# anuragranj/cc

Measured on AMD Instinct MI355X. Metric: train images/sec (832x256, 5-frame sample, 6-scale CC step), higher is better.
Workload: dtype f32; 1 GPU; full CC: DispResNet6+PoseNetB6+MaskNet6+Back2Future, all losses; per_gpu_batch=4, global_batch=4, height=256, width=832, scales=6, frames=5, parallelism=dp1, hipgraph=True, trained_nets=all, rccl_ranks=1, dead_occlusion_decoders_elided=False, net_streams=2, pipeline=per_network, grad_chunks=False, deterministic=True

## Files before the change

### cc_amd/csrc/wgrad_thin.hip

```cpp
#include <stdio.h>
#include <type_traits>
#include <stdlib.h>
#include "cc_common.h"
#include "conv_internal.h"
#include "cc_tools.h"

namespace {

typedef float f32x4 __attribute__((ext_vector_type(4)));

constexpr int THIN_NW = 4;

struct WT {
    const float* a; const float* x; float* ws;
    int B, M, AH, AW; long a_bs;
    int Cin, IH, IW; long x_bs;
    int R, nxc, units, upb, npb, ngc, ngt, swz;
};

template <int S, int SI, int PAD, int TR>
struct ThinCfg {
    static constexpr int PQ = (PAD + 3) / 4;
    static constexpr int IMAX = SI * 3 + S - 1 - PAD + 4 * PQ;
    static constexpr int NQ = IMAX / 4 + 1;
    static constexpr int TS = TR * S;
};

template <int S, int SI, int PAD, int TR, int DBG>
__device__ __forceinline__ void wgrad_thin_body(const WT& g, const int bx_, const int by_) {
    typedef ThinCfg<S, SI, PAD, TR> C;
    constexpr int PQ = C::PQ, NQ = C::NQ, TS = C::TS;
    __shared__ float red[TS * 256];
    const int lane = threadIdx.x & 63;
    const int wave = __builtin_amdgcn_readfirstlane((int)(threadIdx.x >> 6));
    const int i = lane & 15, k = lane >> 4;
    int combo = by_;
    const int tg = combo % g.ngt;
    combo /= g.ngt;
    const int cg = combo % g.ngc, mg = combo / g.ngc;
    const int r0 = tg * TR;
    const int m = mg * 16 + i, c = cg * 16 + i;
    const bool mok = m < g.M, cok = c < g.Cin;
    const float* __restrict__ abase = g.a + (long)(mok ? m : 0) * g.AH * g.AW;
    const float* __restrict__ xbase = g.x + (long)(cok ? c : 0) * g.IH * g.IW;

    f32x4 acc[TR][S];
#pragma unroll
    for (int tr = 0; tr < TR; tr++)
#pragma unroll
        for (int s = 0; s < S; s++) acc[tr][s] = (f32x4){0.f, 0.f, 0.f, 0.f};

    const int pb = (g.swz ? ((bx_ & 7) * (g.npb >> 3) + (bx_ >> 3)) : bx_);
    const int u0 = pb * g.upb;
    const int u1 = (u0 + g.upb < g.units) ? (u0 + g.upb) : g.units;

    constexpr int KEEP = (TR > SI) ? TR - SI : 0;
    float4 An;
    float4 Wn[TR][NQ], Wc[TR][NQ];
    auto issue = [&](auto T0, int b, int y, int xc, float4& A, float4 (&W)[TR][NQ]) {
        constexpr int t0 = decltype(T0)::value;
        const int x0 = xc * 16 + 4 * k;
        const int xa = (x0 < g.AW) ? x0 : 0;
        A = *(const float4*)(abase + (unsigned)(b * (int)g.a_bs + y * g.AW + xa));
        const unsigned xb = (unsigned)(b * (int)g.x_bs);
#pragma unroll
        for (int tr = t0; tr < TR; tr++) {
            int iy = y * SI + r0 + tr - PAD;
            iy = iy < 0 ? 0 : (iy >= g.IH ? g.IH - 1 : iy);
            const unsigned xr = xb + (unsigned)(iy * g.IW);
#pragma unroll
            for (int q = 0; q < NQ; q++) {
                int col = SI * x0 - 4 * PQ + 4 * q;
                col = (col < 0 || col >= g.IW) ? 0 : col;
                W[tr][q] = *(const float4*)(xbase + (xr + (unsigned)col));
            }
        }
    };

    const int ngx = (g.nxc + THIN_NW - 1) / THIN_NW;
    int u = u0;
    const int ue = u1;
    if (u < ue) {
        int nb, ny, nxcpos;
        {
            const int colu = u / g.AH;
            ny = u - colu * g.AH;
            nb = colu / ngx;
            nxcpos = (colu - nb * ngx) * THIN_NW + wave;
        }
        typedef std::integral_constant<int, 0> ALL;
        typedef std::integral_constant<int, KEEP> NEW;
        issue(ALL(), nb, ny, nxcpos, An, Wn);
        bool fresh = true;
        for (; u < ue; u++) {
            const float4 Ac = An;
            if (fresh) {
#pragma unroll
                for (int tr = 0; tr < TR; tr++)
#pragma unroll
                    for (int q = 0; q < NQ; q++) Wc[tr][q] = Wn[tr][q];
            } else {
#pragma unroll
                for (int tr = 0; tr < TR; tr++)
#pragma unroll
                    for (int q = 0; q < NQ; q++) Wc[tr][q] = (tr < KEEP) ? Wc[tr + (TR - KEEP)][q] : Wn[tr][q];
            }
            const int y = ny, xc = nxcpos;
            if (u + 1 < ue) {
                fresh = false;
                if (++ny == g.AH) {
                    ny = 0;
                    fresh = true;
                    nxcpos += THIN_NW;
                    if (nxcpos - wave >= g.nxc) { nxcpos = wave; nb++; }
                }
                if (DBG != 2) {
                    if (fresh) issue(ALL(), nb, ny, nxcpos, An, Wn);
                    else issue(NEW(), nb, ny, nxcpos, An, Wn);
                }
            }

            const int x0 = xc * 16 + 4 * k;
            const bool aok = mok && (x0 < g.AW);
            float a4[4];
            a4[0] = aok ? Ac.x : 0.f;
            a4[1] = aok ? Ac.y : 0.f;
            a4[2] = aok ? Ac.z : 0.f;
            a4[3] = aok ? Ac.w : 0.f;
#pragma unroll
            for (int tr = 0; tr < TR; tr++) {
                const int iy = y * SI + r0 + tr - PAD;
                const bool rok = cok && (r0 + tr < g.R) && iy >= 0 && iy < g.IH;
                float w[NQ * 4];
#pragma unroll
                for (int q = 0; q < NQ; q++) {
                    const int col = SI * x0 - 4 * PQ + 4 * q;
                    const bool ok = rok && col >= 0 && col < g.IW;
                    w[4 * q + 0] = ok ? Wc[tr][q].x : 0.f;
                    w[4 * q + 1] = ok ? Wc[tr][q].y : 0.f;
                    w[4 * q + 2] = ok ? Wc[tr][q].z : 0.f;
                    w[4 * q + 3] = ok ? Wc[tr][q].w : 0.f;
                }
                if (DBG == 1) {
#pragma unroll
                    for (int s = 0; s < S; s++)
#pragma unroll
                        for (int j = 0; j < 4; j++) acc[tr][s][j] += a4[j] * w[SI * j + s - PAD + 4 * PQ];
                    continue;
                }
#pragma unroll
                for (int j = 0; j < 4; j++)
#pragma unroll
                    for (int s = 0; s < S; s++)
                        acc[tr][s] = __builtin_amdgcn_mfma_f32_16x16x4f32(a4[j], w[SI * j + s - PAD + 4 * PQ], acc[tr][s], 0, 0, 0);
            }
        }
    }

#pragma unroll 1
    for (int wv = 0; wv < THIN_NW; wv++) {
        if (wave == wv) {
#pragma unroll
            for (int tr = 0; tr < TR; tr++)
#pragma unroll
                for (int s = 0; s < S; s++)
#pragma unroll
                    for (int r = 0; r < 4; r++) {
                        const int idx = ((tr * S + s) * 4 + r) * 64 + lane;
                        const float v = acc[tr][s][r];
                        red[idx] = (wv == 0) ? v : (red[idx] + v);
                    }
        }
        __syncthreads();
    }
    float* __restrict__ slab = g.ws + ((long)by_ * g.npb + pb) * (TS * 256);
    for (int e = threadIdx.x; e < TS * 256; e += 64 * THIN_NW) {
        const int t = e >> 8, mc = e & 255, mm = mc >> 4, cc_ = mc & 15;
        slab[e] = red[(t * 4 + (mm & 3)) * 64 + (mm >> 2) * 16 + cc_];
    }
}


template <int S, int SI, int PAD, int TR, int DBG = 0>
__global__ __launch_bounds__(64 * THIN_NW) void k_wgrad_thin(WT g) {
    wgrad_thin_body<S, SI, PAD, TR, DBG>(g, (int)blockIdx.x, (int)blockIdx.y);
}

constexpr int THIN_MAXP = 24;
struct WTM { WT p[THIN_MAXP]; int blk_end[THIN_MAXP]; int n; };
template <int S, int SI, int PAD, int TR>
__global__ __launch_bounds__(64 * THIN_NW) void k_wgrad_thin_multi(WTM a) {
    int k = 0, first = 0;
#pragma unroll 1
    for (int q = 0; q + 1 < a.n; q++)
        if ((int)blockIdx.x >= a.blk_end[q]) { k = q + 1; first = a.blk_end[q]; }
#if defined(__HIP_DEVICE_COMPILE__) && !defined(CC_HIPEMU)
    const WT& g = *(reinterpret_cast<const WT*>((const char*)__builtin_amdgcn_kernarg_segment_ptr() + offsetof(WTM, p)) + k);
#else
    const WT& g = a.p[k];
#endif
    const int b = (int)blockIdx.x - first;
    const int by = b / g.npb;
    wgrad_thin_body<S, SI, PAD, TR, 0>(g, b - by * g.npb, by);
}


int env_int(const char* name, int dflt) { return cctools::env_int(name, dflt); }

struct ThinPlan {
    bool ok;
    int kind, TR, ngm, ngc, ngt, nxc, units, upb, npb, TS;
    size_t ws_floats;
};

enum { K_3_1 = 0, K_3_2, K_7_2, K_7_1, K_1_1, K_5_2, K_4_2, K_1_2, K_NONE };

ThinPlan plan_thin(int B, int M, int AH, int AW, int Cin, int R, int S, int si) {
    ThinPlan p = {};
    p.kind = K_NONE;
    if (R != S || env_int("CC_NO_WGRAD_THIN", 0)) return p;
    if (S == 3 && si == 1) { p.kind = K_3_1; p.TR = 3; }
    else if (S == 3 && si == 2) { p.kind = K_3_2; p.TR = 3; }
    else if (S == 7 && si == 2) { p.kind = K_7_2; p.TR = 2; }
    else if (S == 7 && si == 1) { p.kind = K_7_1; p.TR = 2; }
    else if (S == 1 && si == 1) { p.kind = K_1_1; p.TR = 1; }
    else if (S == 5 && si == 2) { p.kind = K_5_2; p.TR = 3; }
    else if (S == 4 && si == 2) { p.kind = K_4_2; p.TR = 4; }
    else if (S == 1 && si == 2) { p.kind = K_1_2; p.TR = 1; }
    else return p;
    p.ngm = (M + 15) / 16;
    p.ngc = (Cin + 15) / 16;
    const long P = (long)B * AH * AW;
    if ((AW & 3) || p.ngm * p.ngc > env_int("CC_WGRAD_THIN_MAXCOMBO", 15) || P < env_int("CC_WGRAD_THIN_MINPIX", 8192) ||
        (S == 7 && Cin < 8)) return p;
    p.ngt = (R + p.TR - 1) / p.TR;
    p.TS = p.TR * S;
    p.nxc = (AW + 15) / 16;
    const long units = (long)B * AH * ((p.nxc + THIN_NW - 1) / THIN_NW);
    if (units > (1l << 30)) return p;
    p.units = (int)units;
    long npb = units / env_int("CC_WGRAD_THIN_UPB", 8);
    const long cap = env_int("CC_WGRAD_THIN_NPB", 256);
    npb = npb < 1 ? 1 : (npb > cap ? cap : npb);
    p.upb = (int)((units + npb - 1) / npb);
    p.npb = (p.units + p.upb - 1) / p.upb;
    if (p.npb >= 64) p.npb = ((p.npb + 7) / 8) * 8;
    p.ws_floats = (size_t)p.ngm * p.ngc * p.ngt * p.npb * p.TS * 256;
    p.ok = true;
    return p;
}

template <int S, int SI, int PAD, int TR>
void launch_thin(const WT& g, dim3 grid, hipStream_t s) {
    hipLaunchKernelGGL(HIP_KERNEL_NAME(k_wgrad_thin<S, SI, PAD, TR>), grid, dim3(64 * THIN_NW), 0, s, g);
}

template <int S, int SI, int PAD, int TR>
void launch_thin_multi(const WTM& m, unsigned blocks, hipStream_t s) {
    hipLaunchKernelGGL(HIP_KERNEL_NAME(k_wgrad_thin_multi<S, SI, PAD, TR>), dim3(blocks), dim3(64 * THIN_NW), 0, s, m);
}

constexpr int THIN_PARK_CAP = 96;
struct ThinParkedOne { WT g; int kind, ncombo; double gflop; };
struct ThinParked { bool on; int n; ThinParkedOne d[THIN_PARK_CAP]; };
thread_local ThinParked g_thin_parked = {};

void launch_thin_kind(int kind, const WT& g, dim3 grid, hipStream_t s) {
    switch (kind) {
        case K_3_1: launch_thin<3, 1, 1, 3>(g, grid, s); break;
        case K_3_2: launch_thin<3, 2, 1, 3>(g, grid, s); break;
        case K_7_2: launch_thin<7, 2, 3, 2>(g, grid, s); break;
        case K_7_1: launch_thin<7, 1, 3, 2>(g, grid, s); break;
        case K_1_1: launch_thin<1, 1, 0, 1>(g, grid, s); break;
        case K_5_2: launch_thin<5, 2, 2, 3>(g, grid, s); break;
        case K_1_2: launch_thin<1, 2, 0, 1>(g, grid, s); break;
        default: launch_thin<4, 2, 1, 4>(g, grid, s); break;
    }
}

void launch_thin_multi_kind(int kind, const WTM& m, unsigned blocks, hipStream_t s) {
    switch (kind) {
        case K_3_1: launch_thin_multi<3, 1, 1, 3>(m, blocks, s); break;
        case K_3_2: launch_thin_multi<3, 2, 1, 3>(m, blocks, s); break;
        case K_7_2: launch_thin_multi<7, 2, 3, 2>(m, blocks, s); break;
        case K_7_1: launch_thin_multi<7, 1, 3, 2>(m, blocks, s); break;
        case K_1_1: launch_thin_multi<1, 1, 0, 1>(m, blocks, s); break;
        case K_5_2: launch_thin_multi<5, 2, 2, 3>(m, blocks, s); break;
        case K_1_2: launch_thin_multi<1, 2, 0, 1>(m, blocks, s); break;
        default: launch_thin_multi<4, 2, 1, 4>(m, blocks, s); break;
    }
}

}

namespace ccint {

bool wgrad_thin_park(bool on) {
    const bool was = g_thin_parked.on;
    g_thin_parked.on = on && !env_int("CC_NO_WGRAD_THIN_LIST", 0);
    return was;
}

bool wgrad_thin_parking() { return g_thin_parked.on; }

double wgrad_thin_parked_gflop() {
    double gf = 0;
    for (int i = 0; i < g_thin_parked.n; i++) gf += g_thin_parked.d[i].gflop;
    return gf;
}

void wgrad_thin_flush(hipStream_t s) {
    ThinParked& P = g_thin_parked;
    for (int kind = 0; kind < K_NONE && P.n > 0; kind++) {
        int i = 0;
        while (i < P.n) {
            WTM m = {};
            long blk = 0;
            int last = -1;
            for (; i < P.n && m.n < THIN_MAXP; i++) {
                if (P.d[i].kind != kind) continue;
                const long nb = (long)P.d[i].g.npb * P.d[i].ncombo;
                if (m.n && blk + nb >= (1l << 31)) break;
                m.p[m.n] = P.d[i].g;
                blk += nb;
                m.blk_end[m.n] = (int)blk;
                m.n++;
                last = i;
            }
            if (!m.n) break;
            if (env_int("CC_WGRAD_THIN_TRACE", 0)) fprintf(stderr, "[wgrad_thin_multi] kind %d: %d problems, %ld workgroups\n", kind, m.n, blk);
            if (m.n == 1) launch_thin_kind(kind, P.d[last].g, dim3((unsigned)P.d[last].g.npb, (unsigned)P.d[last].ncombo), s);
            else launch_thin_multi_kind(kind, m, (unsigned)blk, s);
        }
    }
    P.n = 0;
}

size_t wgrad_thin_ws_floats(int B, int M, int AH, int AW, int Cin, int R, int S, int si) {
    const ThinPlan p = plan_thin(B, M, AH, AW, Cin, R, S, si);
    return p.ok ? p.ws_floats : 0;
}

bool wgrad_thin_launch(const float* a, const float* x, float* gw, float* ws, int B, int M, int AH, int AW, long a_bs, int Cin,
                       int IH, int IW, long x_bs, int R, int S, int si, int pad, long o_sm, long o_sc, int accumulate, hipStream_t s,
                       RedSink* sink) {
    const ThinPlan p = plan_thin(B, M, AH, AW, Cin, R, S, si);
    if (!p.ok || (IW & 3) || (a_bs & 3) || (x_bs & 3) || (((uintptr_t)a | (uintptr_t)x) & 15)) return false;
    if ((long)B * a_bs >= (1l << 31) || (long)B * x_bs >= (1l << 31)) return false;
    static const int want_pad[] = {1, 1, 3, 3, 0, 2, 1, 0};
    if (pad != want_pad[p.kind]) return false;
    WT g = {};
    g.a = a; g.x = x; g.ws = ws;
    g.B = B; g.M = M; g.AH = AH; g.AW = AW; g.a_bs = a_bs; g.Cin = Cin; g.IH = IH; g.IW = IW; g.x_bs = x_bs;
    g.R = R; g.nxc = p.nxc; g.units = p.units; g.upb = p.upb; g.npb = p.npb; g.ngc = p.ngc; g.ngt = p.ngt;
    g.swz = (p.npb % 8 == 0 && p.npb >= 64 && !env_int("CC_WGRAD_THIN_NOSWZ", 0)) ? 1 : 0;
    const int ncombo = p.ngm * p.ngc * p.ngt;
    if (env_int("CC_WGRAD_THIN_TRACE", 0))
        fprintf(stderr, "[wgrad_thin] kind %d M %d Cin %d A %dx%d X %dx%d npb %d upb %d combos %d\n", p.kind, M, Cin, AH, AW, IH, IW,
                p.npb, p.upb, ncombo);
    dim3 grid((unsigned)p.npb, (unsigned)ncombo);
    if (g_thin_parked.on && sink && g_thin_parked.n < THIN_PARK_CAP) {
        ThinParkedOne& d = g_thin_parked.d[g_thin_parked.n++];
        d.g = g; d.kind = p.kind; d.ncombo = ncombo;
        d.gflop = 2e-9 * B * AH * AW * (double)M * Cin * R * S;
        const long rdp[RD_LONGS] = {2, (long)ws, (long)gw, p.npb, accumulate, o_sm, o_sc, p.TS, S, p.TR, p.ngc, p.ngt, M, Cin, R, ncombo};
        (void)wgrad_reduce_emit(sink, rdp, 1, s);
        return true;
    }
    switch (p.kind) {
        case K_3_1: {
            const int dbg = env_int("CC_WGRAD_THIN_DBG", 0);
            if (dbg == 1) hipLaunchKernelGGL(HIP_KERNEL_NAME(k_wgrad_thin<3, 1, 1, 3, 1>), grid, dim3(64 * THIN_NW), 0, s, g);
            else if (dbg == 2) hipLaunchKernelGGL(HIP_KERNEL_NAME(k_wgrad_thin<3, 1, 1, 3, 2>), grid, dim3(64 * THIN_NW), 0, s, g);
            else launch_thin<3, 1, 1, 3>(g, grid, s);
            break;
        }
        case K_3_2: launch_thin<3, 2, 1, 3>(g, grid, s); break;
        case K_7_2: launch_thin<7, 2, 3, 2>(g, grid, s); break;
        case K_7_1: launch_thin<7, 1, 3, 2>(g, grid, s); break;
        case K_1_1: launch_thin<1, 1, 0, 1>(g, grid, s); break;
        case K_5_2: launch_thin<5, 2, 2, 3>(g, grid, s); break;
        case K_1_2: launch_thin<1, 2, 0, 1>(g, grid, s); break;
        default: launch_thin<4, 2, 1, 4>(g, grid, s); break;
    }
    const long rd[RD_LONGS] = {2, (long)ws, (long)gw, p.npb, accumulate, o_sm, o_sc, p.TS, S, p.TR, p.ngc, p.ngt, M, Cin, R, ncombo};
    (void)wgrad_reduce_emit(sink, rd, 1, s);
    return true;
}

void wgrad_thin_name(int B, int M, int AH, int AW, int Cin, int IH, int IW, int R, int S, int si, int pad, char* out, int cap) {
    out[0] = 0;
    const ThinPlan p = plan_thin(B, M, AH, AW, Cin, R, S, si);
    static const int want_pad[] = {1, 1, 3, 3, 0, 2, 1, 0};
    static const int tr[] = {3, 3, 2, 2, 1, 3, 4, 1};
    if (!p.ok || (IW & 3) || pad != want_pad[p.kind]) return;
    snprintf(out, cap, "k_wgrad_thin<%d, %d, %d, %d>", S, si, pad, tr[p.kind]);
}

}
```

Before: 248.1 images/s.

## Process two dY channel groups per wave in thin wgrad to reuse input loads

The thin weight-gradient kernel now lets each workgroup handle two 16-channel output groups (GM=2) for selected kernel kinds. The input rows loaded for the MFMA B-operand are shared across both groups, and the grid is halved in the M dimension. It also restructures row prefetch so kept rows are reloaded only at column changes. This trades higher register pressure, more accumulators and a serialized two-pass LDS reduction for fewer redundant global loads of x.

```diff
diff --git a/cc_amd/csrc/wgrad_thin.hip b/cc_amd/csrc/wgrad_thin.hip
--- a/cc_amd/csrc/wgrad_thin.hip
+++ b/cc_amd/csrc/wgrad_thin.hip
@@ -26,55 +26,54 @@
     static constexpr int TS = TR * S;
 };
 
-template <int S, int SI, int PAD, int TR, int DBG>
-__device__ __forceinline__ void wgrad_thin_body(const WT& g, const int bx_, const int by_) {
+template <int S, int SI, int PAD, int TR, int DBG, int GM, int NG>
+__device__ __forceinline__ void wgrad_thin_units(const WT& g, const int mg0, const int cg, const int r0, const int u0, const int u1,
+                                                 f32x4 (&acc)[GM][TR][S]) {
     typedef ThinCfg<S, SI, PAD, TR> C;
-    constexpr int PQ = C::PQ, NQ = C::NQ, TS = C::TS;
-    __shared__ float red[TS * 256];
+    constexpr int PQ = C::PQ, NQ = C::NQ;
     const int lane = threadIdx.x & 63;
     const int wave = __builtin_amdgcn_readfirstlane((int)(threadIdx.x >> 6));
     const int i = lane & 15, k = lane >> 4;
-    int combo = by_;
-    const int tg = combo % g.ngt;
-    combo /= g.ngt;
-    const int cg = combo % g.ngc, mg = combo / g.ngc;
-    const int r0 = tg * TR;
-    const int m = mg * 16 + i, c = cg * 16 + i;
-    const bool mok = m < g.M, cok = c < g.Cin;
-    const float* __restrict__ abase = g.a + (long)(mok ? m : 0) * g.AH * g.AW;
+    const int c = cg * 16 + i;
+    const bool cok = c < g.Cin;
     const float* __restrict__ xbase = g.x + (long)(cok ? c : 0) * g.IH * g.IW;
-
-    f32x4 acc[TR][S];
-#pragma unroll
-    for (int tr = 0; tr < TR; tr++)
-#pragma unroll
-        for (int s = 0; s < S; s++) acc[tr][s] = (f32x4){0.f, 0.f, 0.f, 0.f};
-
-    const int pb = (g.swz ? ((bx_ & 7) * (g.npb >> 3) + (bx_ >> 3)) : bx_);
-    const int u0 = pb * g.upb;
-    const int u1 = (u0 + g.upb < g.units) ? (u0 + g.upb) : g.units;
+    bool mok[NG];
+    const float* __restrict__ abase[NG];
+#pragma unroll
+    for (int gi = 0; gi < NG; gi++) {
+        const int m = (mg0 + gi) * 16 + i;
+        mok[gi] = m < g.M;
+        abase[gi] = g.a + (long)(mok[gi] ? m : 0) * g.AH * g.AW;
+    }
 
     constexpr int KEEP = (TR > SI) ? TR - SI : 0;
-    float4 An;
-    float4 Wn[TR][NQ], Wc[TR][NQ];
-    auto issue = [&](auto T0, int b, int y, int xc, float4& A, float4 (&W)[TR][NQ]) {
-        constexpr int t0 = decltype(T0)::value;
+    constexpr int NR = TR - KEEP;
+    float4 An[NG];
+    float4 Wn[NR][NQ], Wc[TR][NQ];
+    auto issue_row = [&](int tr, int b, int y, int xc, float4 (&W)[NQ]) {
+        const int x0 = xc * 16 + 4 * k;
+        int iy = y * SI + r0 + tr - PAD;
+        iy = iy < 0 ? 0 : (iy >= g.IH ? g.IH - 1 : iy);
+        const unsigned xr = (unsigned)(b * (int)g.x_bs) + (unsigned)(iy * g.IW);
+#pragma unroll
+        for (int q = 0; q < NQ; q++) {
+            int col = SI * x0 - 4 * PQ + 4 * q;
+            col = (col < 0 || col >= g.IW) ? 0 : col;
+            W[q] = *(const float4*)(xbase + (xr + (unsigned)col));
+        }
+    };
+    auto issue = [&](int b, int y, int xc) {
         const int x0 = xc * 16 + 4 * k;
         const int xa = (x0 < g.AW) ? x0 : 0;
-        A = *(const float4*)(abase + (unsigned)(b * (int)g.a_bs + y * g.AW + xa));
-        const unsigned xb = (unsigned)(b * (int)g.x_bs);
-#pragma unroll
-        for (int tr = t0; tr < TR; tr++) {
-            int iy = y * SI + r0 + tr - PAD;
-            iy = iy < 0 ? 0 : (iy >= g.IH ? g.IH - 1 : iy);
-            const unsigned xr = xb + (unsigned)(iy * g.IW);
-#pragma unroll
-            for (int q = 0; q < NQ; q++) {
-                int col = SI * x0 - 4 * PQ + 4 * q;
-                col = (col < 0 || col >= g.IW) ? 0 : col;
-                W[tr][q] = *(const float4*)(xbase + (xr + (unsigned)col));
-            }
-        }
+        const unsigned ao = (unsigned)(b * (int)g.a_bs + y * g.AW + xa);
+#pragma unroll
+        for (int gi = 0; gi < NG; gi++) An[gi] = *(const float4*)(abase[gi] + ao);
+#pragma unroll
+        for (int tr = KEEP; tr < TR; tr++) issue_row(tr, b, y, xc, Wn[tr - KEEP]);
+    };
+    auto issue_keep = [&](int b, int y, int xc) {
+#pragma unroll
+        for (int tr = 0; tr < KEEP; tr++) issue_row(tr, b, y, xc, Wc[tr + NR]);
     };
 
     const int ngx = (g.nxc + THIN_NW - 1) / THIN_NW;
@@ -88,45 +87,38 @@
             nb = colu / ngx;
             nxcpos = (colu - nb * ngx) * THIN_NW + wave;
         }
-        typedef std::integral_constant<int, 0> ALL;
-        typedef std::integral_constant<int, KEEP> NEW;
-        issue(ALL(), nb, ny, nxcpos, An, Wn);
-        bool fresh = true;
+        issue_keep(nb, ny, nxcpos);
+        issue(nb, ny, nxcpos);
         for (; u < ue; u++) {
-            const float4 Ac = An;
-            if (fresh) {
-#pragma unroll
-                for (int tr = 0; tr < TR; tr++)
-#pragma unroll
-                    for (int q = 0; q < NQ; q++) Wc[tr][q] = Wn[tr][q];
-            } else {
-#pragma unroll
-                for (int tr = 0; tr < TR; tr++)
-#pragma unroll
-                    for (int q = 0; q < NQ; q++) Wc[tr][q] = (tr < KEEP) ? Wc[tr + (TR - KEEP)][q] : Wn[tr][q];
-            }
+            float4 Ac[NG];
+#pragma unroll
+            for (int gi = 0; gi < NG; gi++) Ac[gi] = An[gi];
+#pragma unroll
+            for (int tr = 0; tr < TR; tr++)
+#pragma unroll
+                for (int q = 0; q < NQ; q++) Wc[tr][q] = (tr < KEEP) ? Wc[tr + NR][q] : Wn[tr - KEEP][q];
             const int y = ny, xc = nxcpos;
+            bool fresh = false;
             if (u + 1 < ue) {
-                fresh = false;
                 if (++ny == g.AH) {
                     ny = 0;
                     fresh = true;
                     nxcpos += THIN_NW;
                     if (nxcpos - wave >= g.nxc) { nxcpos = wave; nb++; }
                 }
-                if (DBG != 2) {
-                    if (fresh) issue(ALL(), nb, ny, nxcpos, An, Wn);
-                    else issue(NEW(), nb, ny, nxcpos, An, Wn);
-                }
+                if (DBG != 2) issue(nb, ny, nxcpos);
             }
 
             const int x0 = xc * 16 + 4 * k;
-            const bool aok = mok && (x0 < g.AW);
-            float a4[4];
-            a4[0] = aok ? Ac.x : 0.f;
-            a4[1] = aok ? Ac.y : 0.f;
-            a4[2] = aok ? Ac.z : 0.f;
-            a4[3] = aok ? Ac.w : 0.f;
+            float a4[NG][4];
+#pragma unroll
+            for (int gi = 0; gi < NG; gi++) {
+                const bool aok = mok[gi] && (x0 < g.AW);
+                a4[gi][0] = aok ? Ac[gi].x : 0.f;
+                a4[gi][1] = aok ? Ac[gi].y : 0.f;
+                a4[gi][2] = aok ? Ac[gi].z : 0.f;
+                a4[gi][3] = aok ? Ac[gi].w : 0.f;
+            }
 #pragma unroll
             for (int tr = 0; tr < TR; tr++) {
                 const int iy = y * SI + r0 + tr - PAD;
@@ -141,54 +133,94 @@
                     w[4 * q + 2] = ok ? Wc[tr][q].z : 0.f;
                     w[4 * q + 3] = ok ? Wc[tr][q].w : 0.f;
                 }
-                if (DBG == 1) {
+#pragma unroll
+                for (int gi = 0; gi < NG; gi++) {
+                    if (DBG == 1) {
+#pragma unroll
+                        for (int s = 0; s < S; s++)
+#pragma unroll
+                            for (int j = 0; j < 4; j++) acc[gi][tr][s][j] += a4[gi][j] * w[SI * j + s - PAD + 4 * PQ];
+                        continue;
+                    }
+#pragma unroll
+                    for (int j = 0; j < 4; j++)
+#pragma unroll
+                        for (int s = 0; s < S; s++)
+                            acc[gi][tr][s] =
+                                __builtin_amdgcn_mfma_f32_16x16x4f32(a4[gi][j], w[SI * j + s - PAD + 4 * PQ], acc[gi][tr][s], 0, 0, 0);
+                }
+            }
+            if (KEEP > 0 && DBG != 2 && fresh) issue_keep(nb, ny, nxcpos);
+        }
+    }
+}
+
+template <int S, int SI, int PAD, int TR, int DBG, int GM>
+__device__ __forceinline__ void wgrad_thin_body(const WT& g, const int bx_, const int by_) {
+    typedef ThinCfg<S, SI, PAD, TR> C;
+    constexpr int TS = C::TS;
+    static_assert(GM == 1 || GM == 2, "one or two dY channel groups per wave");
+    __shared__ float red[TS * 256];
+    const int lane = threadIdx.x & 63;
+    const int wave = __builtin_amdgcn_readfirstlane((int)(threadIdx.x >> 6));
+    int combo = by_;
+    const int tg = combo % g.ngt;
+    combo /= g.ngt;
+    const int cg = combo % g.ngc, mg0 = (combo / g.ngc) * GM;
+    const int ng = (GM > 1 && mg0 + 1 < (g.M + 15) / 16) ? GM : 1;
+
+    f32x4 acc[GM][TR][S];
+#pragma unroll
+    for (int gi = 0; gi < GM; gi++)
+#pragma unroll
+        for (int tr = 0; tr < TR; tr++)
+#pragma unroll
+            for (int s = 0; s < S; s++) acc[gi][tr][s] = (f32x4){0.f, 0.f, 0.f, 0.f};
+
+    const int pb = (g.swz ? ((bx_ & 7) * (g.npb >> 3) + (bx_ >> 3)) : bx_);
+    const int u0 = pb * g.upb;
+    const int u1 = (u0 + g.upb < g.units) ? (u0 + g.upb) : g.units;
+
+    if (GM > 1 && ng == GM) wgrad_thin_units<S, SI, PAD, TR, DBG, GM, GM>(g, mg0, cg, tg * TR, u0, u1, acc);
+    else wgrad_thin_units<S, SI, PAD, TR, DBG, GM, 1>(g, mg0, cg, tg * TR, u0, u1, acc);
+
+#pragma unroll
+    for (int gi = 0; gi < GM; gi++) {
+        if (gi >= ng) break;
+        if (gi) __syncthreads();
+#pragma unroll 1
+        for (int wv = 0; wv < THIN_NW; wv++) {
+            if (wave == wv) {
+#pragma unroll
+                for (int tr = 0; tr < TR; tr++)
 #pragma unroll
                     for (int s = 0; s < S; s++)
 #pragma unroll
-                        for (int j = 0; j < 4; j++) acc[tr][s][j] += a4[j] * w[SI * j + s - PAD + 4 * PQ];
-                    continue;
-                }
-#pragma unroll
-                for (int j = 0; j < 4; j++)
-#pragma unroll
-                    for (int s = 0; s < S; s++)
-                        acc[tr][s] = __builtin_amdgcn_mfma_f32_16x16x4f32(a4[j], w[SI * j + s - PAD + 4 * PQ], acc[tr][s], 0, 0, 0);
+                        for (int r = 0; r < 4; r++) {
+                            const int idx = ((tr * S + s) * 4 + r) * 64 + lane;
+                            const float v = acc[gi][tr][s][r];
+                            red[idx] = (wv == 0) ? v : (red[idx] + v);
+                        }
             }
-        }
-    }
-
-#pragma unroll 1
-    for (int wv = 0; wv < THIN_NW; wv++) {
-        if (wave == wv) {
-#pragma unroll
-            for (int tr = 0; tr < TR; tr++)
-#pragma unroll
-                for (int s = 0; s < S; s++)
-#pragma unroll
-                    for (int r = 0; r < 4; r++) {
-                        const int idx = ((tr * S + s) * 4 + r) * 64 + lane;
-                        const float v = acc[tr][s][r];
-                        red[idx] = (wv == 0) ? v : (red[idx] + v);
-                    }
-        }
-        __syncthreads();
-    }
-    float* __restrict__ slab = g.ws + ((long)by_ * g.npb + pb) * (TS * 256);
-    for (int e = threadIdx.x; e < TS * 256; e += 64 * THIN_NW) {
-        const int t = e >> 8, mc = e & 255, mm = mc >> 4, cc_ = mc & 15;
-        slab[e] = red[(t * 4 + (mm & 3)) * 64 + (mm >> 2) * 16 + cc_];
-    }
-}
-
-
-template <int S, int SI, int PAD, int TR, int DBG = 0>
+            __syncthreads();
+        }
+        float* __restrict__ slab = g.ws + ((((long)(mg0 + gi) * g.ngc + cg) * g.ngt + tg) * g.npb + pb) * (TS * 256);
+        for (int e = threadIdx.x; e < TS * 256; e += 64 * THIN_NW) {
+            const int t = e >> 8, mc = e & 255, mm = mc >> 4, cc_ = mc & 15;
+            slab[e] = red[(t * 4 + (mm & 3)) * 64 + (mm >> 2) * 16 + cc_];
+        }
+    }
+}
+
+
+template <int S, int SI, int PAD, int TR, int DBG = 0, int GM = 1>
 __global__ __launch_bounds__(64 * THIN_NW) void k_wgrad_thin(WT g) {
-    wgrad_thin_body<S, SI, PAD, TR, DBG>(g, (int)blockIdx.x, (int)blockIdx.y);
+    wgrad_thin_body<S, SI, PAD, TR, DBG, GM>(g, (int)blockIdx.x, (int)blockIdx.y);
 }
 
 constexpr int THIN_MAXP = 24;
 struct WTM { WT p[THIN_MAXP]; int blk_end[THIN_MAXP]; int n; };
-template <int S, int SI, int PAD, int TR>
+template <int S, int SI, int PAD, int TR, int GM = 1>
 __global__ __launch_bounds__(64 * THIN_NW) void k_wgrad_thin_multi(WTM a) {
     int k = 0, first = 0;
 #pragma unroll 1
@@ -201,7 +233,7 @@
 #endif
     const int b = (int)blockIdx.x - first;
     const int by = b / g.npb;
-    wgrad_thin_body<S, SI, PAD, TR, 0>(g, b - by * g.npb, by);
+    wgrad_thin_body<S, SI, PAD, TR, 0, GM>(g, b - by * g.npb, by);
 }
 
 
@@ -250,44 +282,54 @@
     return p;
 }
 
+constexpr int THIN_GM_KINDS = (1 << K_3_1) | (1 << K_3_2) | (1 << K_1_2);
+int thin_gm(int kind) {
+    if (env_int("CC_WGRAD_THIN_GM", 2) < 2) return 1;
+    return ((env_int("CC_WGRAD_THIN_GM_KINDS", THIN_GM_KINDS) >> kind) & 1) ? 2 : 1;
+}
+
+int thin_rows(int ngm, int ngc, int ngt, int gm) { return ((ngm + gm - 1) / gm) * ngc * ngt; }
+
 template <int S, int SI, int PAD, int TR>
-void launch_thin(const WT& g, dim3 grid, hipStream_t s) {
-    hipLaunchKernelGGL(HIP_KERNEL_NAME(k_wgrad_thin<S, SI, PAD, TR>), grid, dim3(64 * THIN_NW), 0, s, g);
+void launch_thin(const WT& g, dim3 grid, int gm, hipStream_t s) {
+    if (gm == 2) hipLaunchKernelGGL(HIP_KERNEL_NAME(k_wgrad_thin<S, SI, PAD, TR, 0, 2>), grid, dim3(64 * THIN_NW), 0, s, g);
+    else hipLaunchKernelGGL(HIP_KERNEL_NAME(k_wgrad_thin<S, SI, PAD, TR, 0, 1>), grid, dim3(64 * THIN_NW), 0, s, g);
 }
 
 template <int S, int SI, int PAD, int TR>
-void launch_thin_multi(const WTM& m, unsigned blocks, hipStream_t s) {
-    hipLaunchKernelGGL(HIP_KERNEL_NAME(k_wgrad_thin_multi<S, SI, PAD, TR>), dim3(blocks), dim3(64 * THIN_NW), 0, s, m);
+void launch_thin_multi(const WTM& m, unsigned blocks, int gm, hipStream_t s) {
+    if (gm == 2) hipLaunchKernelGGL(HIP_KERNEL_NAME(k_wgrad_thin_multi<S, SI, PAD, TR, 2>), dim3(blocks), dim3(64 * THIN_NW), 0, s, m);
+    else hipLaunchKernelGGL(HIP_KERNEL_NAME(k_wgrad_thin_multi<S, SI, PAD, TR, 1>), dim3(blocks), dim3(64 * THIN_NW), 0, s, m);
 }
 
 constexpr int THIN_PARK_CAP = 96;
-struct ThinParkedOne { WT g; int kind, ncombo; double gflop; };
+struct ThinParkedOne { WT g; int kind, gm, ncombo; double gflop; };
 struct ThinParked { bool on; int n; ThinParkedOne d[THIN_PARK_CAP]; };
 thread_local ThinParked g_thin_parked = {};
 
-void launch_thin_kind(int kind, const WT& g, dim3 grid, hipStream_t s) {
+void launch_thin_kind(int kind, const WT& g, dim3 grid, int gm, hipStream_t s) {
     switch (kind) {
-        case K_3_1: launch_thin<3, 1, 1, 3>(g, grid, s); break;
-        case K_3_2: launch_thin<3, 2, 1, 3>(g, grid, s); break;
-        case K_7_2: launch_thin<7, 2, 3, 2>(g, grid, s); break;
-        case K_7_1: launch_thin<7, 1, 3, 2>(g, grid, s); break;
-        case K_1_1: launch_thin<1, 1, 0, 1>(g, grid, s); break;
-        case K_5_2: launch_thin<5, 2, 2, 3>(g, grid, s); break;
-        case K_1_2: launch_thin<1, 2, 0, 1>(g, grid, s); break;
-        default: launch_thin<4, 2, 1, 4>(g, grid, s); break;
-    }
-}
-
-void launch_thin_multi_kind(int kind, const WTM& m, unsigned blocks, hipStream_t s) {
+        case K_3_1: launch_thin<3, 1, 1, 3>(g, grid, gm, s); break;
+        case K_3_2: launch_thin<3, 2, 1, 3>(g, grid, gm, s); break;
+        case K_7_2: launch_thin<7, 2, 3, 2>(g, grid, gm, s); break;
+        case K_7_1: launch_thin<7, 1, 3, 2>(g, grid, gm, s); break;
+        case K_1_1: launch_thin<1, 1, 0, 1>(g, grid, gm, s); break;
+        case K_5_2: launch_thin<5, 2, 2, 3>(g, grid, gm, s); break;
+        case K_1_2: launch_thin<1, 2, 0, 1>(g, grid, gm, s); break;
+        default: launch_thin<4, 2, 1, 4>(g, grid, gm, s); break;
+    }
+}
+
+void launch_thin_multi_kind(int kind, const WTM& m, unsigned blocks, int gm, hipStream_t s) {
     switch (kind) {
-        case K_3_1: launch_thin_multi<3, 1, 1, 3>(m, blocks, s); break;
-        case K_3_2: launch_thin_multi<3, 2, 1, 3>(m, blocks, s); break;
-        case K_7_2: launch_thin_multi<7, 2, 3, 2>(m, blocks, s); break;
-        case K_7_1: launch_thin_multi<7, 1, 3, 2>(m, blocks, s); break;
-        case K_1_1: launch_thin_multi<1, 1, 0, 1>(m, blocks, s); break;
-        case K_5_2: launch_thin_multi<5, 2, 2, 3>(m, blocks, s); break;
-        case K_1_2: launch_thin_multi<1, 2, 0, 1>(m, blocks, s); break;
-        default: launch_thin_multi<4, 2, 1, 4>(m, blocks, s); break;
+        case K_3_1: launch_thin_multi<3, 1, 1, 3>(m, blocks, gm, s); break;
+        case K_3_2: launch_thin_multi<3, 2, 1, 3>(m, blocks, gm, s); break;
+        case K_7_2: launch_thin_multi<7, 2, 3, 2>(m, blocks, gm, s); break;
+        case K_7_1: launch_thin_multi<7, 1, 3, 2>(m, blocks, gm, s); break;
+        case K_1_1: launch_thin_multi<1, 1, 0, 1>(m, blocks, gm, s); break;
+        case K_5_2: launch_thin_multi<5, 2, 2, 3>(m, blocks, gm, s); break;
+        case K_1_2: launch_thin_multi<1, 2, 0, 1>(m, blocks, gm, s); break;
+        default: launch_thin_multi<4, 2, 1, 4>(m, blocks, gm, s); break;
     }
 }
 
@@ -311,14 +353,15 @@
 
 void wgrad_thin_flush(hipStream_t s) {
     ThinParked& P = g_thin_parked;
-    for (int kind = 0; kind < K_NONE && P.n > 0; kind++) {
+    for (int inst = 0; inst < 2 * K_NONE && P.n > 0; inst++) {
+        const int kind = inst >> 1, gm = 1 + (inst & 1);
         int i = 0;
         while (i < P.n) {
             WTM m = {};
             long blk = 0;
             int last = -1;
             for (; i < P.n && m.n < THIN_MAXP; i++) {
-                if (P.d[i].kind != kind) continue;
+                if (P.d[i].kind != kind || P.d[i].gm != gm) continue;
                 const long nb = (long)P.d[i].g.npb * P.d[i].ncombo;
                 if (m.n && blk + nb >= (1l << 31)) break;
                 m.p[m.n] = P.d[i].g;
@@ -328,9 +371,9 @@
                 last = i;
             }
             if (!m.n) break;
-            if (env_int("CC_WGRAD_THIN_TRACE", 0)) fprintf(stderr, "[wgrad_thin_multi] kind %d: %d problems, %ld workgroups\n", kind, m.n, blk);
-            if (m.n == 1) launch_thin_kind(kind, P.d[last].g, dim3((unsigned)P.d[last].g.npb, (unsigned)P.d[last].ncombo), s);
-            else launch_thin_multi_kind(kind, m, (unsigned)blk, s);
+            if (env_int("CC_WGRAD_THIN_TRACE", 0)) fprintf(stderr, "[wgrad_thin_multi] kind %d gm %d: %d problems, %ld workgroups\n", kind, gm, m.n, blk);
+            if (m.n == 1) launch_thin_kind(kind, P.d[last].g, dim3((unsigned)P.d[last].g.npb, (unsigned)P.d[last].ncombo), gm, s);
+            else launch_thin_multi_kind(kind, m, (unsigned)blk, gm, s);
         }
     }
     P.n = 0;
@@ -355,13 +398,17 @@
     g.R = R; g.nxc = p.nxc; g.units = p.units; g.upb = p.upb; g.npb = p.npb; g.ngc = p.ngc; g.ngt = p.ngt;
     g.swz = (p.npb % 8 == 0 && p.npb >= 64 && !env_int("CC_WGRAD_THIN_NOSWZ", 0)) ? 1 : 0;
     const int ncombo = p.ngm * p.ngc * p.ngt;
+    const bool park = g_thin_parked.on && sink && g_thin_parked.n < THIN_PARK_CAP;
+    const int dbg = (p.kind == K_3_1 && !park) ? env_int("CC_WGRAD_THIN_DBG", 0) : 0;
+    const int gm = (dbg == 1 || dbg == 2) ? 1 : thin_gm(p.kind);
+    const int rows = thin_rows(p.ngm, p.ngc, p.ngt, gm);
     if (env_int("CC_WGRAD_THIN_TRACE", 0))
-        fprintf(stderr, "[wgrad_thin] kind %d M %d Cin %d A %dx%d X %dx%d npb %d upb %d combos %d\n", p.kind, M, Cin, AH, AW, IH, IW,
-                p.npb, p.upb, ncombo);
-    dim3 grid((unsigned)p.npb, (unsigned)ncombo);
-    if (g_thin_parked.on && sink && g_thin_parked.n < THIN_PARK_CAP) {
+        fprintf(stderr, "[wgrad_thin] kind %d M %d Cin %d A %dx%d X %dx%d npb %d upb %d combos %d gm %d rows %d\n", p.kind, M, Cin, AH, AW,
+                IH, IW, p.npb, p.upb, ncombo, gm, rows);
+    dim3 grid((unsigned)p.npb, (unsigned)rows);
+    if (park) {
         ThinParkedOne& d = g_thin_parked.d[g_thin_parked.n++];
-        d.g = g; d.kind = p.kind; d.ncombo = ncombo;
+        d.g = g; d.kind = p.kind; d.gm = gm; d.ncombo = rows;
         d.gflop = 2e-9 * B * AH * AW * (double)M * Cin * R * S;
         const long rdp[RD_LONGS] = {2, (long)ws, (long)gw, p.npb, accumulate, o_sm, o_sc, p.TS, S, p.TR, p.ngc, p.ngt, M, Cin, R, ncombo};
         (void)wgrad_reduce_emit(sink, rdp, 1, s);
@@ -369,19 +416,12 @@
     }
     switch (p.kind) {
         case K_3_1: {
-            const int dbg = env_int("CC_WGRAD_THIN_DBG", 0);
             if (dbg == 1) hipLaunchKernelGGL(HIP_KERNEL_NAME(k_wgrad_thin<3, 1, 1, 3, 1>), grid, dim3(64 * THIN_NW), 0, s, g);
             else if (dbg == 2) hipLaunchKernelGGL(HIP_KERNEL_NAME(k_wgrad_thin<3, 1, 1, 3, 2>), grid, dim3(64 * THIN_NW), 0, s, g);
-            else launch_thin<3, 1, 1, 3>(g, grid, s);
+            else launch_thin<3, 1, 1, 3>(g, grid, gm, s);
             break;
         }
-        case K_3_2: launch_thin<3, 2, 1, 3>(g, grid, s); break;
-        case K_7_2: launch_thin<7, 2, 3, 2>(g, grid, s); break;
-        case K_7_1: launch_thin<7, 1, 3, 2>(g, grid, s); break;
-        case K_1_1: launch_thin<1, 1, 0, 1>(g, grid, s); break;
-        case K_5_2: launch_thin<5, 2, 2, 3>(g, grid, s); break;
-        case K_1_2: launch_thin<1, 2, 0, 1>(g, grid, s); break;
-        default: launch_thin<4, 2, 1, 4>(g, grid, s); break;
+        default: launch_thin_kind(p.kind, g, grid, gm, s); break;
     }
     const long rd[RD_LONGS] = {2, (long)ws, (long)gw, p.npb, accumulate, o_sm, o_sc, p.TS, S, p.TR, p.ngc, p.ngt, M, Cin, R, ncombo};
     (void)wgrad_reduce_emit(sink, rd, 1, s);
```

Measured after the change: 249.9 images/s (median of 6 runs). Within noise of the previous version (+0.7%).
